# moddyz/stereo-to-multiview-cuda

Measured on AMD Instinct MI355X. Metric: stereo->8-view frames/sec @1080p d=64; cost-agg HBM GB/s vs roofline, higher is better.
Workload: dtype f32; 1 GPU; 1920x1080 synthetic stereo frame, D=64, zd=32, full stereo->8-view frame: cost init + cross aggregation + WTA + DCC/IRV x5/bilateral + 6 DIBR views + interlacing, one frame per GPU per step; stages=3, usd=34, lsd=17, views=8, aggregation=matrix pipe (stm_kernels_aggm.hip)

## Files before the change

### stereo-to-multiview-cuda_amd/csrc/stm_kernels_agg.hip

```cpp
#include "stm_hwin.h"

namespace stm {

constexpr uint32_t W10_ONE = 1u | (1u << 10) | (1u << 20);
constexpr uint32_t W10_GUARD = 512u * W10_ONE;

__global__ __launch_bounds__(256) void stm_k_widen_px(const uint32_t *__restrict__ bgrx, uint32_t *__restrict__ wide, int n)
{
    const int i = blockIdx.x * 256 + threadIdx.x;
    if (i >= n) return;
    const uint32_t p = bgrx[i];
    wide[i] = (p & 0xffu) | ((p & 0xff00u) << 2) | ((p & 0xff0000u) << 4);
}


struct ArmsArgs {
    const uint32_t *img[2];
    u8 *up[2], *down[2], *left[2], *right[2];
    uint32_t *htab;
    uint32_t *vtab;
    int vrec, vtop;
};

template <int MODE>
__global__ __launch_bounds__(MODE == 2 ? 1024 : 256) void stm_k_cross_arms(ArmsArgs a, uint32_t tg_far, uint32_t tg_near, int usd, int lsd, int H, int W)
{
    constexpr bool HTAB = MODE >= 1;
    const int v = blockIdx.z;
    const int wv_ = __builtin_amdgcn_readfirstlane((int)(threadIdx.x >> 6));
    const int xr = MODE == 2 ? blockIdx.x * 64 + (threadIdx.x & 63) : blockIdx.x * 256 + threadIdx.x;
    const int yr = MODE == 2 ? blockIdx.y * 16 + wv_ : blockIdx.y;
    if (MODE == 1 ? (xr & ~63) >= W : MODE == 0 ? xr >= W : false) return;
    const int x = min(xr, W - 1), y = min(yr, H - 1);
    const int p = y * W + x;
    const uint32_t *__restrict__ img = a.img[v];
    const uint32_t anchor = img[p];
    const char *rowbase = (const char *)img + (size_t)y * W * 4;
    const uint32_t x4 = 4u * (uint32_t)x;
    const int xmax4 = 4 * (W - 1);
    const size_t rowb = (size_t)W * 4;
    const int kmax[4] = {min(usd, y), min(usd, H - 1 - y), min(usd, x), min(usd, W - 1 - x)};
#define STM_ARM_LOADS(K)                                                                                         \
    {                                                                                                            \
        uint32_t xo = x4;                                                                                        \
        asm volatile("" : "+v"(xo));  \
        c[0] = *(const uint32_t *)(rowbase - (size_t)min(K, kmax[0]) * rowb + (size_t)xo);                        \
        c[1] = *(const uint32_t *)(rowbase + (size_t)min(K, kmax[1]) * rowb + (size_t)xo);                        \
        c[2] = *(const uint32_t *)(rowbase + (size_t)(uint32_t)max((int)x4 - 4 * (K), 0));                        \
        c[3] = *(const uint32_t *)(rowbase + (size_t)(uint32_t)min((int)x4 + 4 * (K), xmax4));                    \
    }
    int arm[4] = {kmax[0], kmax[1], kmax[2], kmax[3]};
    const uint32_t anchor_n = anchor + tg_near;
    uint32_t prev[4] = {anchor, anchor, anchor, anchor}, prev_t[4] = {anchor_n, anchor_n, anchor_n, anchor_n};
    int k = 1;
    const int knear = min(usd, lsd);
    while (k <= knear) {
        if (__ballot(k <= max(max(arm[0], arm[1]), max(arm[2], arm[3]))) == 0) break;
#pragma unroll
        for (int j = 0; j < 2; ++j) {
            if (k <= knear) {
                uint32_t c[4];
                STM_ARM_LOADS(k)
#pragma unroll
                for (int d = 0; d < 4; ++d) {
                    const uint32_t c_t = c[d] + tg_near;
                    const uint32_t ok = (c_t - anchor) & (anchor_n - c[d]) & (c_t - prev[d]) & (prev_t[d] - c[d]) & W10_GUARD;
                    arm[d] = min(arm[d], ok != W10_GUARD ? k : 0x7fffffff);
                    prev[d] = c[d];
                    prev_t[d] = c_t;
                }
                ++k;
            }
        }
    }
    const uint32_t far_lo = tg_far - anchor, far_hi = anchor + tg_far;
    k = max(k, knear + 1);
    while (k <= usd) {
        if (__ballot(k <= max(max(arm[0], arm[1]), max(arm[2], arm[3]))) == 0) break;
#pragma unroll
        for (int j = 0; j < 2; ++j) {
            if (k <= usd) {
                uint32_t c[4];
                STM_ARM_LOADS(k)
#pragma unroll
                for (int d = 0; d < 4; ++d) {
                    const uint32_t ok = (c[d] + far_lo) & (far_hi - c[d]) & W10_GUARD;
                    arm[d] = min(arm[d], ok != W10_GUARD ? k : 0x7fffffff);
                }
                ++k;
            }
        }
    }
#undef STM_ARM_LOADS
    const bool inside = xr < W && yr < H;
    if (inside) {
        a.up[v][p] = (u8)arm[0];
        a.down[v][p] = (u8)arm[1];
        a.left[v][p] = (u8)arm[2];
        a.right[v][p] = (u8)arm[3];
    }
    if (HTAB) {
        __shared__ uint32_t ev_all[MODE == 2 ? 16 : 4][4 * 96];
        const int nTx = (W + 15) >> 4;
        if (yr < H)
            hwin_build(a.htab + (size_t)v * H * nTx * HR_REC, ev_all[wv_], yr, xr & ~63, arm[2], arm[3], W, nTx);
    }
    if (MODE == 2) {
        __shared__ u8 s_u[16][64], s_d[16][64];
        __shared__ unsigned long long ev_v[16][96];
        const int l = threadIdx.x & 63;
        s_u[wv_][l] = inside ? (u8)arm[0] : (u8)0;
        s_d[wv_][l] = inside ? (u8)arm[1] : (u8)0;
        __syncthreads();
        const int G = (W + 3) >> 2, nT = (H + 15) >> 4, gg = blockIdx.x * 16 + wv_, u = blockIdx.y;
        if (gg < G) {
            const int b = l >> 4, i = l & 15;
            const int aU = s_u[i][4 * wv_ + b], aD = s_d[i][4 * wv_ + b];
            vwin_build(a.vtab + ((size_t)(v * nT + u) * G + gg) * a.vrec, ev_v[wv_], u, a.vtop, blockIdx.y * 16 + i - aU, aU + aD);
        }
    }
}

static uint32_t wide_threshold(float t)
{
    int ti;
    if (t != t) ti = 255;
    else if (t >= 255.f) ti = 255;
    else if (t < 0.f) ti = -1;
    else ti = (int)floorf(t);
    return (uint32_t)(512 + ti) * W10_ONE;
}

void launch_cross_arms2(int nviews, const uint32_t *const *packed, u8 *const *up, u8 *const *down, u8 *const *left,
                        u8 *const *right, float ucd, float lcd, int usd, int lsd, int H, int W, const uint32_t *const *wide_ready,
                        uint32_t *htab, uint32_t *vtab, int vrec, int vtop)
{
    ArmsArgs a;
    const int n = H * W;
    ProfScope p("cross_arms");
    const uint32_t *wide[2];
    for (int v = 0; v < nviews; ++v) {
        if (wide_ready) {
            wide[v] = wide_ready[v];
            continue;
        }
        uint32_t *w = Workspace::get<uint32_t>((size_t)n);
        STM_LAUNCH(stm_k_widen_px, dim3(cdiv(n, 256)), dim3(256), 0, stream(), packed[v], w, n);
        STM_CHECK_LAUNCH();
        wide[v] = w;
    }
    for (int v = 0; v < 2; ++v) {
        const int s = v < nviews ? v : 0;
        a.img[v] = wide[s]; a.up[v] = up[s]; a.down[v] = down[s]; a.left[v] = left[s]; a.right[v] = right[s];
    }
    if (usd > 255) usd = 255;
    a.htab = htab;
    a.vtab = vtab;
    a.vrec = vrec;
    a.vtop = vtop;
    if (htab && vtab && vtop >= 0 && usd <= HR_TOP && usd <= vtop)
        STM_LAUNCH(stm_k_cross_arms<2>, dim3(cdiv(W, 64), cdiv(H, 16), nviews), dim3(1024), 0, stream(), a, wide_threshold(ucd),
                           wide_threshold(lcd), usd, lsd, H, W);
    else if (htab && usd <= HR_TOP)
        STM_LAUNCH(stm_k_cross_arms<1>, dim3(cdiv(W, 256), H, nviews), dim3(256), 0, stream(), a, wide_threshold(ucd),
                           wide_threshold(lcd), usd, lsd, H, W);
    else
        STM_LAUNCH(stm_k_cross_arms<0>, dim3(cdiv(W, 256), H, nviews), dim3(256), 0, stream(), a, wide_threshold(ucd),
                           wide_threshold(lcd), usd, lsd, H, W);
    STM_CHECK_LAUNCH();
}

void launch_cross_arms(const uint32_t *packed, u8 *up, u8 *down, u8 *left, u8 *right, float ucd, float lcd, int usd,
                       int lsd, int H, int W)
{
    launch_cross_arms2(1, &packed, &up, &down, &left, &right, ucd, lcd, usd, lsd, H, W, nullptr);
}

#define STM_ACC(s, v) { s.x = s.x + v.x; s.y = s.y + v.y; s.z = s.z + v.z; s.w = s.w + v.w; }

template <int S> __device__ __forceinline__ float4 window_sum(const float4 *__restrict__ p, int n, float4 s)
{
    while (n >= 4) {
        float4 v0 = p[0], v1 = p[S], v2 = p[2 * S], v3 = p[3 * S];
        p += 4 * S;
        n -= 4;
        STM_ACC(s, v0) STM_ACC(s, v1) STM_ACC(s, v2) STM_ACC(s, v3)
    }
    if (n & 2) {
        float4 v0 = p[0], v1 = p[S];
        p += 2 * S;
        STM_ACC(s, v0) STM_ACC(s, v1)
    }
    if (n & 1) {
        float4 v0 = p[0];
        STM_ACC(s, v0)
    }
    return s;
}

static void allow_lds(const void *func, size_t bytes)
{
    if (bytes > 64 * 1024) STM_CHECK(hipFuncSetAttribute(func, hipFuncAttributeMaxDynamicSharedMemorySize, (int)bytes));
}

constexpr int AH_QPB = 4;

struct AggHView {
    Vol in, out;
    const u8 *armL, *armR;
    float *disp;
    const uint32_t *pk_own, *cen_own, *pk_oth, *cen_oth;
    int sgn;
};

__device__ __forceinline__ int hamdist_low32(uint32_t a, uint32_t b)
{
    const uint32_t x = a ^ b;
    return __popc(x & 0x7fffffffu) + 33 * (int)(x >> 31);
}

template <bool QUAD, bool WTA, int T, int PPT, bool COST = false>
__global__ __launch_bounds__(T) void stm_k_agg_h(Vol in, Vol out, const u8 *__restrict__ armL,
                                                 const u8 *__restrict__ armR, float *__restrict__ disp,
                                                 int D, int zd, int H, int W, int qpb, AggHView first, AggHView second,
                                                 const float *__restrict__ lut_g)
{
    const AggHView &vw = blockIdx.z ? second : first;
    if (blockIdx.z) {
        in = second.in;
        out = second.out;
        armL = second.armL;
        armR = second.armR;
        disp = second.disp;
    }
    extern __shared__ float4 smem4[];
    float4 *tile = smem4;
    uint16_t *arms = (uint16_t *)(tile + W);
    const int y = blockIdx.x, tid = threadIdx.x;
    const size_t row = (size_t)y * W;
    const int nq = (D + 3) >> 2;
    const int q0 = blockIdx.y * qpb, q1 = min(q0 + qpb, nq);

    for (int x = tid; x < W; x += T) arms[x] = (uint16_t)armL[row + x] | ((uint16_t)armR[row + x] << 8);

    float *lut_ad = (float *)(arms + ((W + 1) & ~1));
    float *lut_c = lut_ad + 768;
    uint32_t pk0[COST ? PPT : 1], cen0[COST ? PPT : 1];
    if (COST) {
        for (int i = tid; i < 768 + 65; i += T) lut_ad[i] = lut_g[i];
#pragma unroll
        for (int i = 0; i < PPT; ++i) {
            const int x = min(tid + i * T, W - 1);
            pk0[i] = vw.pk_own[row + x];
            cen0[i] = vw.cen_own[row + x];
        }
        __syncthreads();
    }
    const uint32_t *__restrict__ pk_oth = vw.pk_oth + row, *__restrict__ cen_oth = vw.cen_oth + row;
    const int sgn = vw.sgn;
    typedef uint32_t u32x4 __attribute__((ext_vector_type(4), aligned(4)));
    auto cost_quad = [&](int q, int x, uint32_t p0, uint32_t c0) {
        float v[4];
        const int xb = x + sgn * (q * 4 - zd), xe = xb + 3 * sgn;
        const int lo = min(xb, xe);
        const bool edge = lo < 0 || lo + 3 > W - 1 || q * 4 + 3 >= D;
        if (__builtin_amdgcn_ballot_w64(edge) == 0) {
            const u32x4 pp = *(const u32x4 *)(pk_oth + lo), cc = *(const u32x4 *)(cen_oth + lo);
#pragma unroll
            for (int j = 0; j < 4; ++j) {
                const uint32_t p1 = sgn > 0 ? pp[j] : pp[3 - j], c1 = sgn > 0 ? cc[j] : cc[3 - j];
                const int ad = (int)__builtin_amdgcn_sad_u8(p0, p1, 0u);
                const int hd = hamdist_low32(c0, c1);
                v[j] = lut_ad[ad] + lut_c[hd];
            }
            return make_float4(v[0], v[1], v[2], v[3]);
        }
#pragma unroll
        for (int j = 0; j < 4; ++j) {
            const int d = q * 4 + j;
            v[j] = 0.f;
            if (d < D) {
                const int xo = min(max(x + sgn * (d - zd), 0), W - 1);
                const int ad = (int)__builtin_amdgcn_sad_u8(p0, pk_oth[xo], 0u);
                const int hd = hamdist_low32(c0, cen_oth[xo]);
                v[j] = lut_ad[ad] + lut_c[hd];
            }
        }
        return make_float4(v[0], v[1], v[2], v[3]);
    };

    float4 pre[PPT];
    float best_c[WTA ? PPT : 1];
    int best_d[WTA ? PPT : 1];
#pragma unroll
    for (int i = 0; i < PPT; ++i) {
        const int x = tid + i * T;
        if (x < W) pre[i] = COST ? cost_quad(q0, x, pk0[COST ? i : 0], cen0[COST ? i : 0]) : load_quad<QUAD>(in, q0, D, row + x);
        if (WTA) { best_c[i] = 3.402823466e+38f; best_d[i] = 0; }
    }
    for (int q = q0; q < q1; ++q) {
        __syncthreads();
#pragma unroll
        for (int i = 0; i < PPT; ++i) {
            const int x = tid + i * T;
            if (x < W) tile[x] = pre[i];
        }
        __syncthreads();
        if (q + 1 < q1) {
#pragma unroll
            for (int i = 0; i < PPT; ++i) {
                const int x = tid + i * T;
                if (x < W) pre[i] = COST ? cost_quad(q + 1, x, pk0[COST ? i : 0], cen0[COST ? i : 0]) : load_quad<QUAD>(in, q + 1, D, row + x);
            }
        }
        const int d0 = q * 4;
#pragma unroll
        for (int i = 0; i < PPT; ++i) {
            const int x = tid + i * T;
            if (x < W) {
                const uint32_t ar = arms[x];
                const int aL = (int)(ar & 0xff), n = aL + (int)(ar >> 8);
                const float4 s = window_sum<1>(tile + (x - aL), n, make_float4(0.f, 0.f, 0.f, 0.f));
                if (WTA) {
                    float bc = best_c[i];
                    int bd = best_d[i];
                    if (bc > s.x) { bc = s.x; bd = d0; }
                    if (d0 + 1 < D && bc > s.y) { bc = s.y; bd = d0 + 1; }
                    if (d0 + 2 < D && bc > s.z) { bc = s.z; bd = d0 + 2; }
                    if (d0 + 3 < D && bc > s.w) { bc = s.w; bd = d0 + 3; }
                    best_c[i] = bc;
                    best_d[i] = bd;
                } else {
                    store_quad<QUAD>(out, q, D, row + x, s);
                }
            }
        }
    }
    if (WTA) {
#pragma unroll
        for (int i = 0; i < PPT; ++i) {
            const int x = tid + i * T;
            if (x < W) disp[row + x] = (float)best_d[i] - (float)zd;
        }
    }
}

static size_t agg_h_smem(int W, bool cost = false) { return (size_t)W * 16 + (size_t)((W + 1) & ~1) * 2 + (cost ? (768 + 72) * 4 : 0); }

template <bool QUAD, bool WTA, int T, int PPT, bool COST = false>
static void launch_agg_h_tt(Vol in, Vol out, const u8 *armL, const u8 *armR, float *disp, int D, int zd, int H, int W, int qpb,
                            const AggHView *first, const AggHView *second, const float *lut)
{
    int nq = (D + 3) / 4;
    size_t smem = agg_h_smem(W, COST);
    allow_lds((const void *)stm_k_agg_h<QUAD, WTA, T, PPT, COST>, smem);
    AggHView none{in, out, armL, armR, disp, nullptr, nullptr, nullptr, nullptr, 0};
    STM_LAUNCH((stm_k_agg_h<QUAD, WTA, T, PPT, COST>), dim3(H, cdiv(nq, qpb), second ? 2 : 1), dim3(T), smem, stream(), in,
                       out, armL, armR, disp, D, zd, H, W, qpb, first ? *first : none, second ? *second : none, lut);
    STM_CHECK_LAUNCH();
}

template <bool QUAD, bool WTA, bool COST = false>
static void launch_agg_h_t(Vol in, Vol out, const u8 *armL, const u8 *armR, float *disp, int D, int zd, int H, int W, int qpb,
                           const AggHView *second = nullptr, const AggHView *first = nullptr, const float *lut = nullptr)
{
    const int hv = (agg_variant() / 100) % 10;
    if (W > 8192) {
        fail("aggregation: num_cols > 8192 is not supported by the row-tile kernel", "W", __FILE__, __LINE__);
        return;
    }
    if (hv == 1 && W <= 2048) launch_agg_h_tt<QUAD, WTA, 256, 8, COST>(in, out, armL, armR, disp, D, zd, H, W, qpb, first, second, lut);
    else if (hv == 2 && W <= 2048) launch_agg_h_tt<QUAD, WTA, 1024, 2, COST>(in, out, armL, armR, disp, D, zd, H, W, qpb, first, second, lut);
    else if (W <= 1024) launch_agg_h_tt<QUAD, WTA, 256, 4, COST>(in, out, armL, armR, disp, D, zd, H, W, qpb, first, second, lut);
    else if (W <= 2048) launch_agg_h_tt<QUAD, WTA, 512, 4, COST>(in, out, armL, armR, disp, D, zd, H, W, qpb, first, second, lut);
    else if (W <= 4096) launch_agg_h_tt<QUAD, WTA, 1024, 4, COST>(in, out, armL, armR, disp, D, zd, H, W, qpb, first, second, lut);
    else launch_agg_h_tt<QUAD, WTA, 1024, 8, COST>(in, out, armL, armR, disp, D, zd, H, W, qpb, first, second, lut);
}

void launch_agg_h(Vol in, Vol out, const u8 *armL, const u8 *armR, int D, int H, int W)
{
    ProfScope p("agg_h");
    if (in.quad) launch_agg_h_t<true, false>(in, out, armL, armR, nullptr, D, 0, H, W, AH_QPB);
    else launch_agg_h_t<false, false>(in, out, armL, armR, nullptr, D, 0, H, W, AH_QPB);
}

void launch_agg_h2(Vol in_a, Vol out_a, const u8 *armL_a, const u8 *armR_a, Vol in_b, Vol out_b, const u8 *armL_b, const u8 *armR_b,
                   int D, int H, int W)
{
    ProfScope p("agg_h");
    const AggHView second{in_b, out_b, armL_b, armR_b, nullptr, nullptr, nullptr, nullptr, nullptr, 0};
    if (in_a.quad) launch_agg_h_t<true, false>(in_a, out_a, armL_a, armR_a, nullptr, D, 0, H, W, AH_QPB, &second);
    else launch_agg_h_t<false, false>(in_a, out_a, armL_a, armR_a, nullptr, D, 0, H, W, AH_QPB, &second);
}

void launch_agg_h2_cost(const uint32_t *pk_l, const uint32_t *cen_l, const uint32_t *pk_r, const uint32_t *cen_r, const float *lut,
                        Vol out_l, const u8 *armL_l, const u8 *armR_l, Vol out_r, const u8 *armL_r, const u8 *armR_r, int D, int zd,
                        int H, int W)
{
    ProfScope p("agg_h");
    const AggHView first{out_l, out_l, armL_l, armR_l, nullptr, pk_l, cen_l, pk_r, cen_r, 1};
    const AggHView second{out_r, out_r, armL_r, armR_r, nullptr, pk_r, cen_r, pk_l, cen_l, -1};
    launch_agg_h_t<true, false, true>(out_l, out_l, armL_l, armR_l, nullptr, D, zd, H, W, AH_QPB, &second, &first, lut);
}

void launch_agg_h_wta2(Vol in_a, const u8 *armL_a, const u8 *armR_a, float *disp_a, Vol in_b, const u8 *armL_b, const u8 *armR_b,
                       float *disp_b, int D, int zd, int H, int W)
{
    int nq = (D + 3) / 4;
    Vol none = vol_slab(nullptr, 0);
    const AggHView second{in_b, none, armL_b, armR_b, disp_b, nullptr, nullptr, nullptr, nullptr, 0};
    ProfScope p("agg_hw");
    if (in_a.quad) launch_agg_h_t<true, true>(in_a, none, armL_a, armR_a, disp_a, D, zd, H, W, nq, &second);
    else launch_agg_h_t<false, true>(in_a, none, armL_a, armR_a, disp_a, D, zd, H, W, nq, &second);
}

template <bool QUAD, int TX, int TY, int OPT>
__global__ __launch_bounds__(TX *TY) void stm_k_agg_v(Vol in, Vol out, const u8 *__restrict__ armU,
                                                      const u8 *__restrict__ armD, int D, int H, int W, int usd, int R,
                                                      int band, int nstrips, int nbands, int nq, int xcd_map)
{
    constexpr int CH = TY * OPT;
    extern __shared__ float4 ring[];
    const int tx = threadIdx.x, ty = threadIdx.y;
    int strip, bandi, q;
    {
        const int b = blockIdx.x;
        int tile;
        if (xcd_map) {
            const int xcd = b & 7, i = b >> 3;
            q = i % nq;
            tile = (i / nq) * 8 + xcd;
        } else {
            tile = b % (nstrips * nbands);
            q = b / (nstrips * nbands);
        }
        if (tile >= nstrips * nbands) return;
        strip = tile % nstrips;
        bandi = tile / nstrips;
    }
    const int x = strip * TX + tx;
    const int yb0 = bandi * band, yb1 = min(yb0 + band, H);
    const bool xin = x < W;
    const float4 zero4 = make_float4(0.f, 0.f, 0.f, 0.f);

    const int first = max(yb0 - usd, 0);
    const int slot_first = first % R;
    int loaded = min(yb0 + usd - 1, H);
    if (loaded < first) loaded = first;
    for (int r = first + ty; r < loaded; r += TY) {
        int s = slot_first + (r - first);
        if (s >= R) s -= R;
        ring[s * TX + tx] = xin ? load_quad<QUAD>(in, q, D, (size_t)r * W + x) : zero4;
    }
    int slot_loaded = slot_first + (loaded - first);
    if (slot_loaded >= R) slot_loaded -= R;
    int slot_y0 = yb0 % R;

    float4 pre[OPT];
#pragma unroll
    for (int i = 0; i < OPT; ++i) {
        const int r = loaded + ty + i * TY;
        pre[i] = (xin && r < H) ? load_quad<QUAD>(in, q, D, (size_t)r * W + x) : zero4;
    }
    for (int y0 = yb0; y0 < yb1; y0 += CH) {
        __syncthreads();
#pragma unroll
        for (int i = 0; i < OPT; ++i) {
            const int r = loaded + ty + i * TY;
            int s = slot_loaded + ty + i * TY;
            if (s >= R) s -= R;
            if (r < H) ring[s * TX + tx] = pre[i];
        }
        loaded += CH;
        slot_loaded += CH;
        if (slot_loaded >= R) slot_loaded -= R;
        __syncthreads();
        if (y0 + CH < yb1) {
#pragma unroll
            for (int i = 0; i < OPT; ++i) {
                const int r = loaded + ty + i * TY;
                if (xin && r < H) pre[i] = load_quad<QUAD>(in, q, D, (size_t)r * W + x);
            }
        }
#pragma unroll
        for (int i = 0; i < OPT; ++i) {
            const int y = y0 + ty + i * TY;
            if (xin && y < yb1) {
                const size_t p = (size_t)y * W + x;
                const int aU = (int)armU[p], n = aU + (int)armD[p];
                int sa = slot_y0 + ty + i * TY - aU;
                if (sa < 0) sa += R;
                const int n1 = min(n, R - sa);
                float4 s = window_sum<TX>(ring + sa * TX + tx, n1, zero4);
                s = window_sum<TX>(ring + tx, n - n1, s);
                store_quad<QUAD>(out, q, D, p, s);
            }
        }
        slot_y0 += CH;
        if (slot_y0 >= R) slot_y0 -= R;
    }
}

template <bool QUAD, int TX, int TY, int OPT>
static void launch_agg_v_t(Vol in, Vol out, const u8 *armU, const u8 *armD, int D, int H, int W, int usd, int nbands)
{
    constexpr int CH = TY * OPT;
    int nq = (D + 3) / 4;
    int R = (2 * usd + CH - 1) / CH * CH + CH;
    size_t smem = (size_t)R * TX * 16;
    int band = (cdiv(H, nbands) + CH - 1) / CH * CH;
    if (band < CH) band = CH;
    allow_lds((const void *)stm_k_agg_v<QUAD, TX, TY, OPT>, smem);
    const int nstrips = cdiv(W, TX), nb = cdiv(H, band);
    const int xcd_map = (agg_variant() / 1000) % 10 == 1 ? 0 : 1;
    const int ntiles8 = cdiv(nstrips * nb, 8) * 8;
    STM_LAUNCH((stm_k_agg_v<QUAD, TX, TY, OPT>), dim3((unsigned)ntiles8 * nq), dim3(TX, TY), smem, stream(), in, out,
                       armU, armD, D, H, W, usd, R, band, nstrips, nb, nq, xcd_map);
    STM_CHECK_LAUNCH();
}

void launch_agg_v(Vol in, Vol out, const u8 *armU, const u8 *armD, int D, int H, int W, int usd)
{
    ProfScope p("agg_v");
    const int v = agg_variant() % 100;
    const int nbands = (v / 10) ? (v / 10) : 3;
    if (in.quad) {
        switch (v % 10) {
        default: launch_agg_v_t<true, 16, 32, 1>(in, out, armU, armD, D, H, W, usd, nbands); break;
        case 1: launch_agg_v_t<true, 32, 8, 2>(in, out, armU, armD, D, H, W, usd, nbands); break;
        case 2: launch_agg_v_t<true, 32, 8, 4>(in, out, armU, armD, D, H, W, usd, nbands); break;
        case 3: launch_agg_v_t<true, 16, 16, 2>(in, out, armU, armD, D, H, W, usd, nbands); break;
        case 4: launch_agg_v_t<true, 16, 16, 4>(in, out, armU, armD, D, H, W, usd, nbands); break;
        case 5: launch_agg_v_t<true, 64, 4, 4>(in, out, armU, armD, D, H, W, usd, nbands); break;
        case 6: launch_agg_v_t<true, 16, 16, 1>(in, out, armU, armD, D, H, W, usd, nbands); break;
        case 7: launch_agg_v_t<true, 16, 8, 1>(in, out, armU, armD, D, H, W, usd, nbands); break;
        case 8: launch_agg_v_t<true, 16, 32, 1>(in, out, armU, armD, D, H, W, usd, nbands); break;
        case 9: launch_agg_v_t<true, 8, 32, 1>(in, out, armU, armD, D, H, W, usd, nbands); break;
        }
    } else {
        launch_agg_v_t<false, 32, 16, 1>(in, out, armU, armD, D, H, W, usd, nbands);
    }
}

__global__ __launch_bounds__(256) void stm_k_wta(Vol cost, float *__restrict__ disp, int D, int zd, size_t HW)
{
    size_t p = (size_t)blockIdx.x * 256 + threadIdx.x;
    if (p >= HW) return;
    float lowest = 3.402823466e+38f;
    int best = 0;
    if (cost.quad) {
        for (int q = 0; q * 4 < D; ++q) {
            float4 c = ((const float4 *)cost.base)[(size_t)q * cost.plane_stride + p];
            if (lowest > c.x) { lowest = c.x; best = q * 4; }
            if (q * 4 + 1 < D && lowest > c.y) { lowest = c.y; best = q * 4 + 1; }
            if (q * 4 + 2 < D && lowest > c.z) { lowest = c.z; best = q * 4 + 2; }
            if (q * 4 + 3 < D && lowest > c.w) { lowest = c.w; best = q * 4 + 3; }
        }
    } else {
        for (int d = 0; d < D; ++d) {
            float c = cost.plane(d)[p];
            if (lowest > c) { lowest = c; best = d; }
        }
    }
    disp[p] = (float)best - (float)zd;
}

void launch_wta(Vol cost, float *disp, int D, int zd, int H, int W)
{
    size_t HW = (size_t)H * W;
    ProfScope p("wta");
    STM_LAUNCH(stm_k_wta, dim3((unsigned)((HW + 255) / 256)), dim3(256), 0, stream(), cost, disp, D, zd, HW);
    STM_CHECK_LAUNCH();
}

}
```

Measured before the change: 612.4 frames/s.

## Add multi-segment cross-arm kernel with wave-ballot arm walking and buffer loads

```diff
diff --git a/stereo-to-multiview-cuda_amd/csrc/stm_kernels_agg.hip b/stereo-to-multiview-cuda_amd/csrc/stm_kernels_agg.hip
--- a/stereo-to-multiview-cuda_amd/csrc/stm_kernels_agg.hip
+++ b/stereo-to-multiview-cuda_amd/csrc/stm_kernels_agg.hip
@@ -1,4 +1,5 @@
 #include "stm_hwin.h"
+#include <type_traits>
 
 namespace stm {
 
@@ -121,6 +122,221 @@
     }
 }
 
+#ifndef CA_S_EXP
+#define CA_S_EXP 2
+#endif
+constexpr int CA_S = CA_S_EXP;
+
+
+template <int S, bool TABLES>
+__global__ __launch_bounds__(1024) void stm_k_cross_arms_pairs(ArmsArgs a, uint32_t tg_far, uint32_t tg_near, int usd, int lsd, int H, int W)
+{
+    typedef unsigned long long u64;
+    const int v = blockIdx.z;
+    const int wv_ = __builtin_amdgcn_readfirstlane((int)(threadIdx.x >> 6));
+    const int l = threadIdx.x & 63;
+    const int x0 = blockIdx.x * (64 * S);
+    const int yr = blockIdx.y * 16 + wv_;
+    const bool row_in = yr < H;
+    if (!TABLES && !row_in) return;
+    int armU[S], armD[S], armL[S], armR[S];
+#pragma unroll
+    for (int s = 0; s < S; ++s) armU[s] = armD[s] = armL[s] = armR[s] = 0;
+    if (row_in) {
+        const uint32_t *__restrict__ img = a.img[v];
+        const int y = yr, xmax = W - 1;
+        const char *rowbase = (const char *)img + (size_t)y * W * 4;
+        const uint32_t tf_near = 1023u * W10_ONE - tg_near, tf_far = 1023u * W10_ONE - tg_far;
+        const int knear = max(min(usd, lsd), 0);
+        const int kmaxU = min(usd, y), kmaxD = min(usd, H - 1 - y);
+        const bool halo = x0 > 0;
+        uint32_t anc[S + 1], xc[S];
+        u64 inrow[S];
+#pragma unroll
+        for (int s = 0; s < S; ++s) {
+            const int x = x0 + 64 * s + l;
+            xc[s] = 4u * (uint32_t)min(x, xmax);
+            anc[s] = *(const uint32_t *)(rowbase + xc[s]);
+            inrow[s] = __ballot(x < W);
+        }
+        const int xh = (halo ? x0 - 64 : x0) + l;
+        anc[S] = *(const uint32_t *)(rowbase + 4u * (uint32_t)min(xh, xmax));
+        int adjL[S], adjR[S];
+#pragma unroll
+        for (int s = 0; s < S; ++s) adjL[s] = adjR[s] = 0x7fffffff;
+        if (knear >= 1) {
+            u64 NA[S + 2];
+#pragma unroll
+            for (int i = 0; i < S + 2; ++i) {
+                const int x = x0 + 64 * (i - 1) + l;
+                const uint32_t cur = i >= 1 && i <= S ? anc[i - 1] : *(const uint32_t *)(rowbase + 4u * (uint32_t)min(max(x, 0), xmax));
+                const uint32_t prv = *(const uint32_t *)(rowbase + 4u * (uint32_t)min(max(x - 1, 0), xmax));
+                NA[i] = __ballot((((prv + tf_near) - cur) | ((cur + tf_near) - prv)) & W10_GUARD);
+            }
+#pragma unroll
+            for (int s = 0; s < S; ++s) {
+                const u64 above = ((NA[s + 1] >> 1) >> l) | ((NA[s + 2] << 1) << (62 - l));
+                const u64 below = (NA[s + 1] << (63 - l)) | ((NA[s] >> 1) >> l);
+                const int r = above ? __ffsll(above) : 0x7fffffff, q = below ? __clzll(below) + 1 : 0x7fffffff;
+                adjR[s] = r <= lsd ? r : 0x7fffffff;
+                adjL[s] = q <= lsd ? q : 0x7fffffff;
+            }
+        }
+        u64 aliveU[S], aliveD[S], aliveL[S], aliveR[S];
+        int endU[S], endD[S], endL[S], endR[S];
+        uint32_t hi[S + 1], lo[S + 1], prevU[S], prevD[S], prevUt[S], prevDt[S];
+#pragma unroll
+        for (int s = 0; s < S; ++s) {
+            aliveU[s] = aliveD[s] = aliveL[s] = aliveR[s] = inrow[s];
+            endU[s] = endD[s] = endL[s] = endR[s] = 1;
+            prevU[s] = prevD[s] = anc[s];
+            prevUt[s] = prevDt[s] = anc[s] + tf_near;
+        }
+#pragma unroll
+        for (int s = 0; s <= S; ++s) { hi[s] = anc[s] + tf_near; lo[s] = tf_near - anc[s]; }
+        const bool safe = kmaxU == usd && kmaxD == usd && (size_t)y * W + (size_t)(x0 + 64 * S - 1 + max(usd, 0)) < (size_t)H * W;
+        const uint32_t xo = 4u * (uint32_t)(x0 + l), xoh = 4u * (uint32_t)xh;
+        const u64 no_halo = halo ? 0ull : ~0ull;
+        const __amdgpu_buffer_rsrc_t plane = __builtin_amdgcn_make_buffer_rsrc((void *)img, 0, (uint32_t)H * (uint32_t)W * 4u, 0x00020000);
+        const uint32_t row32 = (uint32_t)W * 4u, so_row = (uint32_t)y * row32;
+        uint32_t so_u = so_row, so_d = so_row, so_h = so_row;
+        auto live = [&](int k, auto near_c, auto safe_c) -> bool {
+            constexpr bool NEAR = decltype(near_c)::value, SAFE = decltype(safe_c)::value;
+            u64 m = 0ull, mu = 0ull, md = 0ull;
+#pragma unroll
+            for (int s = 0; s < S; ++s) {
+                if (NEAR) {
+                    aliveL[s] &= __ballot(adjL[s] >= k);
+                    aliveR[s] &= __ballot(adjR[s] >= k);
+                }
+                m |= aliveL[s] | aliveR[s]; mu |= aliveU[s]; md |= aliveD[s];
+            }
+            if (SAFE) return (m | mu | md) != 0ull;
+            return (m | (k <= kmaxU ? mu : 0ull) | (k <= kmaxD ? md : 0ull)) != 0ull;
+        };
+        auto step = [&](int k, auto near_c, auto safe_c) {
+            constexpr bool NEAR = decltype(near_c)::value, SAFE = decltype(safe_c)::value;
+            if (SAFE || k <= kmaxU) so_u -= row32;
+            if (SAFE || k <= kmaxD) so_d += row32;
+            so_h += 4u;
+            uint32_t ch[S + 1], cu[S], cd[S];
+#pragma unroll
+            for (int s = 0; s < S; ++s) {
+                cu[s] = __builtin_amdgcn_raw_buffer_load_b32(plane, xc[s], so_u, 0);
+                cd[s] = __builtin_amdgcn_raw_buffer_load_b32(plane, xc[s], so_d, 0);
+                ch[s] = SAFE ? __builtin_amdgcn_raw_buffer_load_b32(plane, xo + 256u * s, so_h, 0)
+                             : __builtin_amdgcn_raw_buffer_load_b32(plane, 4u * (uint32_t)min(x0 + 64 * s + l + k, xmax), so_row, 0);
+            }
+            ch[S] = SAFE ? __builtin_amdgcn_raw_buffer_load_b32(plane, xoh, so_h, 0)
+                         : __builtin_amdgcn_raw_buffer_load_b32(plane, 4u * (uint32_t)min(xh + k, xmax), so_row, 0);
+            u64 M[S + 1];
+            M[0] = __ballot(((hi[S] - ch[S]) | (ch[S] + lo[S])) & W10_GUARD) | no_halo;
+#pragma unroll
+            for (int s = 0; s < S; ++s) M[s + 1] = __ballot(((hi[s] - ch[s]) | (ch[s] + lo[s])) & W10_GUARD);
+            const int k1 = k + 1;
+#pragma unroll
+            for (int s = 0; s < S; ++s) {
+                aliveR[s] &= ~M[s + 1];
+                aliveL[s] &= ~((M[s + 1] << k) | (M[s] >> (64 - k)));
+                endR[s] = __builtin_amdgcn_inverse_ballot_w64(aliveR[s]) ? k1 : endR[s];
+                endL[s] = __builtin_amdgcn_inverse_ballot_w64(aliveL[s]) ? k1 : endL[s];
+                uint32_t bu = (hi[s] - cu[s]) | (cu[s] + lo[s]), bd = (hi[s] - cd[s]) | (cd[s] + lo[s]);
+                if (NEAR) {
+                    const uint32_t cut = cu[s] + tf_near, cdt = cd[s] + tf_near;
+                    bu |= (prevUt[s] - cu[s]) | (cut - prevU[s]);
+                    bd |= (prevDt[s] - cd[s]) | (cdt - prevD[s]);
+                    prevU[s] = cu[s]; prevUt[s] = cut;
+                    prevD[s] = cd[s]; prevDt[s] = cdt;
+                }
+                aliveU[s] &= ~__ballot(bu & W10_GUARD);
+                aliveD[s] &= ~__ballot(bd & W10_GUARD);
+                endU[s] = __builtin_amdgcn_inverse_ballot_w64(aliveU[s]) ? k1 : endU[s];
+                endD[s] = __builtin_amdgcn_inverse_ballot_w64(aliveD[s]) ? k1 : endD[s];
+            }
+        };
+        auto walk = [&](auto safe_c) {
+            int k = 1, kend = usd;
+            if (knear & 1) { step(k, std::true_type{}, safe_c); ++k; }
+            while (k <= knear) {
+                if (!live(k, std::true_type{}, safe_c)) { kend = 0; break; }
+                step(k, std::true_type{}, safe_c);
+                step(k + 1, std::true_type{}, safe_c);
+                k += 2;
+            }
+#pragma unroll
+            for (int s = 0; s <= S; ++s) { hi[s] = anc[s] + tf_far; lo[s] = tf_far - anc[s]; }
+#pragma unroll
+            for (int s = 0; s < S; ++s) {
+                aliveL[s] &= __ballot(adjL[s] == 0x7fffffff);
+                aliveR[s] &= __ballot(adjR[s] == 0x7fffffff);
+            }
+            if (k <= kend && ((kend - k) & 1) == 0) { step(k, std::false_type{}, safe_c); ++k; }
+            while (k <= kend) {
+                if (!live(k, std::false_type{}, safe_c)) break;
+                step(k, std::false_type{}, safe_c);
+                step(k + 1, std::false_type{}, safe_c);
+                k += 2;
+            }
+        };
+        if (safe) walk(std::true_type{});
+        else walk(std::false_type{});
+#pragma unroll
+        for (int s = 0; s < S; ++s) {
+            const int x = x0 + 64 * s + l;
+            armU[s] = min(kmaxU, endU[s]);
+            armD[s] = min(kmaxD, endD[s]);
+            armL[s] = min(min(usd, x), min(endL[s], adjL[s]));
+            armR[s] = min(min(usd, xmax - x), min(endR[s], adjR[s]));
+        }
+    }
+    typedef const ArmsArgs __attribute__((address_space(4))) *ArmsArgsK;
+    ArmsArgsK late = (ArmsArgsK)__builtin_amdgcn_kernarg_segment_ptr();
+    asm volatile("" : "+s"(late));
+    if (row_in) {
+        u8 *const up = late->up[v], *const down = late->down[v], *const left = late->left[v], *const right = late->right[v];
+        const size_t prow = (size_t)yr * W;
+#pragma unroll
+        for (int s = 0; s < S; ++s) {
+            const int x = x0 + 64 * s + l;
+            if (x < W) {
+                up[prow + x] = (u8)armU[s];
+                down[prow + x] = (u8)armD[s];
+                left[prow + x] = (u8)armL[s];
+                right[prow + x] = (u8)armR[s];
+            }
+        }
+    }
+    if (TABLES) {
+        __shared__ unsigned long long ev_lds[16][4 * 96 / 2];
+        __shared__ u8 s_u[S][16][64], s_d[S][16][64];
+        uint32_t(*ev_all)[4 * 96] = (uint32_t(*)[4 * 96]) ev_lds;
+        unsigned long long(*ev_v)[4 * 96 / 2] = ev_lds;
+        const int nTx = (W + 15) >> 4;
+#pragma unroll
+        for (int s = 0; s < S; ++s) {
+            const bool inside = row_in && x0 + 64 * s + l < W;
+            if (row_in && x0 + 64 * s < W) {
+                hwin_build(a.htab + (size_t)v * H * nTx * HR_REC, ev_all[wv_], yr, x0 + 64 * s, armL[s], armR[s], W, nTx);
+                __builtin_amdgcn_wave_barrier();
+            }
+            s_u[s][wv_][l] = inside ? (u8)armU[s] : (u8)0;
+            s_d[s][wv_][l] = inside ? (u8)armD[s] : (u8)0;
+        }
+        __syncthreads();
+        const int G = (W + 3) >> 2, nT = (H + 15) >> 4, u = blockIdx.y;
+        const int b = l >> 4, i = l & 15;
+#pragma unroll
+        for (int s = 0; s < S; ++s) {
+            const int gg = (blockIdx.x * S + s) * 16 + wv_;
+            if (gg < G) {
+                const int aU = s_u[s][i][4 * wv_ + b], aD = s_d[s][i][4 * wv_ + b];
+                vwin_build(a.vtab + ((size_t)(v * nT + u) * G + gg) * a.vrec, ev_v[wv_], u, a.vtop, blockIdx.y * 16 + i - aU, aU + aD);
+                __builtin_amdgcn_wave_barrier();
+            }
+        }
+    }
+}
+
 static uint32_t wide_threshold(float t)
 {
     int ti;
@@ -158,7 +374,15 @@
     a.vtab = vtab;
     a.vrec = vrec;
     a.vtop = vtop;
-    if (htab && vtab && vtop >= 0 && usd <= HR_TOP && usd <= vtop)
+    const bool pairs = usd <= HR_TOP && (size_t)H * W < ((size_t)1 << 30) && (agg_variant() / 100) % 10 != 7;
+    const bool both = htab && vtab && vtop >= 0 && usd <= HR_TOP && usd <= vtop;
+    if (both && pairs)
+        STM_LAUNCH((stm_k_cross_arms_pairs<CA_S, true>), dim3(cdiv(W, 64 * CA_S), cdiv(H, 16), nviews), dim3(1024), 0, stream(), a, wide_threshold(ucd),
+                           wide_threshold(lcd), usd, lsd, H, W);
+    else if (!htab && pairs)
+        STM_LAUNCH((stm_k_cross_arms_pairs<CA_S, false>), dim3(cdiv(W, 64 * CA_S), cdiv(H, 16), nviews), dim3(1024), 0, stream(), a, wide_threshold(ucd),
+                           wide_threshold(lcd), usd, lsd, H, W);
+    else if (both)
         STM_LAUNCH(stm_k_cross_arms<2>, dim3(cdiv(W, 64), cdiv(H, 16), nviews), dim3(1024), 0, stream(), a, wide_threshold(ucd),
                            wide_threshold(lcd), usd, lsd, H, W);
     else if (htab && usd <= HR_TOP)
```

Measured after the change: 605.3 frames/s. 1.2% lower.
